# WeebLabs/DSPi

Measured on NVIDIA H100. Metric: audio samples/sec (whole box) at 65536ch x 10-band EQ, 96 kHz; % HBM roofline, higher is better.
Workload: dtype f32

## Files before the change

### dspi_b200/csrc/dspi_common.cuh

```cuda
#pragma once
#ifdef __CUDACC_RTC__
typedef unsigned char uint8_t;
typedef unsigned short uint16_t;
typedef unsigned int uint32_t;
typedef int int32_t;
typedef unsigned long long uint64_t;
typedef long long int64_t;
typedef unsigned long long size_t_rtc;
struct alignas(64) CUtensorMap { unsigned long long opaque[16]; };
#else
#include <cuda.h>
#include <cuda_runtime.h>
#include <stdint.h>
#endif

namespace dspi {

__device__ __forceinline__ uint32_t smem_u32(const void *p)
{
    return static_cast<uint32_t>(__cvta_generic_to_shared(p));
}

__device__ __forceinline__ void mbar_init(uint64_t *bar, uint32_t count)
{
// ... 64 lines not shown
template <int N>
__device__ __forceinline__ void tma_store_wait_read()
{
    asm volatile("cp.async.bulk.wait_group.read %0;" ::"n"(N) : "memory");
}
template <int N>
__device__ __forceinline__ void tma_store_wait_all()
{
    asm volatile("cp.async.bulk.wait_group %0;" ::"n"(N) : "memory");
}

__device__ __forceinline__ void cp_async_4(void *smem_dst, const void *gsrc)
{
    asm volatile("cp.async.ca.shared.global [%0], [%1], 4;" ::"r"(smem_u32(smem_dst)), "l"(gsrc) : "memory");
}
__device__ __forceinline__ void cp_async_commit()
{
    asm volatile("cp.async.commit_group;" ::: "memory");
}
template <int N>
__device__ __forceinline__ void cp_async_wait()
{
    asm volatile("cp.async.wait_group %0;" ::"n"(N) : "memory");
}
__device__ __forceinline__ void cp_async_wait_all()
{
    asm volatile("cp.async.wait_group 0;" ::: "memory");
}
__device__ __forceinline__ void prefetch_tmap(const CUtensorMap *map)
{
    asm volatile("prefetch.tensormap [%0];" ::"l"(reinterpret_cast<uint64_t>(map)) : "memory");
}

}
```

### dspi_b200/csrc/engine.cu

```cuda
#include <cstdarg>
#include <cstdio>
#include <cstdlib>
#include <cstring>
#include <algorithm>
#include <new>
#include <utility>
#include <vector>
#include <sched.h>
#include <unistd.h>
#include <sys/syscall.h>

#include "eq_kernels.cuh"
#include "eq_jit.h"
#include "response.cuh"

namespace {

thread_local char g_err[512] = "";

int fail(int code, const char *fmt, ...)
{
    va_list ap;
    va_start(ap, fmt);
    vsnprintf(g_err, sizeof(g_err), fmt, ap);
// ... 20 lines not shown
        if (cudaGetDriverEntryPoint("cuTensorMapEncodeTiled", &p, cudaEnableDefault, &q) == cudaSuccess && q == cudaDriverEntryPointSuccess)
            fn = reinterpret_cast<EncodeTiledFn>(p);
    }
    return fn;
}

constexpr int kHostBufs = 8;

}

namespace dspi {
char *error_buffer(size_t *cap)
{
    *cap = sizeof(g_err);
    return g_err;
}
}

struct dspi_eq {
    dspi_eq_desc desc;
    int cpl;
    uint32_t rows;
    uint32_t n_groups;
    uint32_t c_pad;
    cudaStream_t stream, s_h2d, s_d2h;
    cudaStream_t s_k[kHostBufs];
    cudaEvent_t ev_begin;
    void *d_aos;
    void *d_coef;
    uint64_t *d_modes;
    uint64_t *d_modes_eff;
    const uint8_t *d_skip;
    uint32_t *d_sched;
    int n_sms;
    size_t aos_elem;
    uint64_t launches;
    void *d_stage[kHostBufs];
    size_t stage_bytes;
    cudaEvent_t ev_in[kHostBufs], ev_done[kHostBufs], ev_out[kHostBufs];
    CUtensorMap tmap;
    void *tm_ptr;
    uint32_t tm_T, tm_ld, tm_rows;
    bool sig_dirty;
    bool sig_stale;
    void *jit;
    char kinfo[320];
    dspi::ResponseBuffers resp;
};

static size_t sched_words(const dspi_eq *e) { return 2 * (size_t)(e->c_pad / 32) + 1; }

extern "C" {

const char *dspi_last_error(void) { return g_err; }

int dspi_device_count(void)
{
    int n = 0;
    if (cudaGetDeviceCount(&n) != cudaSuccess) { cudaGetLastError(); return 0; }
    int ok = 0;
    for (int i = 0; i < n; i++) {
        int major = 0;
        if (cudaDeviceGetAttribute(&major, cudaDevAttrComputeCapabilityMajor, i) == cudaSuccess && major == 9) ok++;
    }
    return ok;
}
// ... 92 lines not shown
    if (!e) return fail(DSPI_ENOMEM, "host allocation failed");
    memset(e, 0, sizeof(*e));
    e->desc = *desc;
    e->sig_dirty = true;
    const bool q28 = desc->arith == DSPI_ARITH_Q28;
    e->cpl = 1;
    if (const char *v = getenv("DSPI_F32_CPL")) e->cpl = atoi(v) == 2 ? 2 : 1;
    if (q28) e->cpl = 1;
    e->rows = 32u * e->cpl;
    e->n_groups = (desc->n_channels + e->rows - 1) / e->rows;
    e->c_pad = e->n_groups * e->rows;
    e->aos_elem = q28 ? sizeof(dspi_biquad_q28) : sizeof(dspi_biquad_f32);

    cudaError_t err;
    const size_t aos_bytes = (size_t)e->c_pad * DSPI_MAX_BANDS * e->aos_elem;
    const size_t coef_bytes = q28 ? (size_t)e->n_groups * DSPI_MAX_BANDS * 20 * 32 * 4 : (size_t)e->c_pad * DSPI_MAX_BANDS * 8 * 4;
    if ((err = cudaStreamCreateWithFlags(&e->stream, cudaStreamNonBlocking)) != cudaSuccess) goto cuda_fail;
    if ((err = cudaStreamCreateWithFlags(&e->s_h2d, cudaStreamNonBlocking)) != cudaSuccess) goto cuda_fail;
    if ((err = cudaStreamCreateWithFlags(&e->s_d2h, cudaStreamNonBlocking)) != cudaSuccess) goto cuda_fail;
    if ((err = cudaEventCreateWithFlags(&e->ev_begin, cudaEventDisableTiming)) != cudaSuccess) goto cuda_fail;
    for (int i = 0; i < kHostBufs; i++) {
        if ((err = cudaStreamCreateWithFlags(&e->s_k[i], cudaStreamNonBlocking)) != cudaSuccess) goto cuda_fail;
        if ((err = cudaEventCreateWithFlags(&e->ev_in[i], cudaEventDisableTiming)) != cudaSuccess) goto cuda_fail;
        if ((err = cudaEventCreateWithFlags(&e->ev_done[i], cudaEventDisableTiming)) != cudaSuccess) goto cuda_fail;
        if ((err = cudaEventCreateWithFlags(&e->ev_out[i], cudaEventDisableTiming)) != cudaSuccess) goto cuda_fail;
    }
    if ((err = cudaMalloc(&e->d_aos, aos_bytes)) != cudaSuccess) goto cuda_fail;
    if ((err = cudaMalloc(&e->d_coef, coef_bytes)) != cudaSuccess) goto cuda_fail;
    if ((err = cudaMemsetAsync(e->d_aos, 0, aos_bytes, e->stream)) != cudaSuccess) goto cuda_fail;
    if ((err = cudaMemsetAsync(e->d_coef, 0, coef_bytes, e->stream)) != cudaSuccess) goto cuda_fail;
    if (!q28) {
        if ((err = cudaMalloc(&e->d_modes, (size_t)e->c_pad * 8)) != cudaSuccess) goto cuda_fail;
        if ((err = cudaMalloc(&e->d_sched, sched_words(e) * 4)) != cudaSuccess) goto cuda_fail;
        if ((err = cudaDeviceGetAttribute(&e->n_sms, cudaDevAttrMultiProcessorCount, desc->device)) != cudaSuccess) goto cuda_fail;
        if ((err = cudaMemsetAsync(e->d_modes, 0, (size_t)e->c_pad * 8, e->stream)) != cudaSuccess) goto cuda_fail;
    }
    if ((err = fill_default_records(e)) != cudaSuccess) goto cuda_fail;
    err = q28 ? dspi::launch_pack_q28((const dspi_biquad_q28 *)e->d_aos, 0, e->c_pad, (int32_t *)e->d_coef, e->stream)
              : dspi::launch_pack_f32((const dspi_biquad_f32 *)e->d_aos, 0, e->c_pad, (float *)e->d_coef, e->d_modes, e->cpl, e->stream);
    if (err != cudaSuccess) goto cuda_fail;
    e->launches++;
    if ((err = cudaStreamSynchronize(e->stream)) != cudaSuccess) goto cuda_fail;
    *out = e;
    return DSPI_OK;

cuda_fail:
    fail(DSPI_ECUDA, "engine setup: %s", cudaGetErrorString(err));
    dspi_eq_destroy(e);
    return err == cudaErrorMemoryAllocation ? DSPI_ENOMEM : DSPI_ECUDA;
}

int dspi_eq_destroy(dspi_eq *e)
{
    if (!e) return DSPI_OK;
    cudaSetDevice(e->desc.device);
    if (e->stream) cudaStreamSynchronize(e->stream);
    if (e->s_h2d) cudaStreamSynchronize(e->s_h2d);
    if (e->s_d2h) cudaStreamSynchronize(e->s_d2h);
    for (int i = 0; i < kHostBufs; i++) {
        if (e->s_k[i]) { cudaStreamSynchronize(e->s_k[i]); cudaStreamDestroy(e->s_k[i]); }
        if (e->d_stage[i]) cudaFree(e->d_stage[i]);
        if (e->ev_in[i]) cudaEventDestroy(e->ev_in[i]);
        if (e->ev_done[i]) cudaEventDestroy(e->ev_done[i]);
        if (e->ev_out[i]) cudaEventDestroy(e->ev_out[i]);
    }
    if (e->d_aos) cudaFree(e->d_aos);
    if (e->d_coef) cudaFree(e->d_coef);
    if (e->d_modes) cudaFree(e->d_modes);
    if (e->d_modes_eff) cudaFree(e->d_modes_eff);
    if (e->d_sched) cudaFree(e->d_sched);
    e->resp.destroy();
    if (e->stream) cudaStreamDestroy(e->stream);
    if (e->s_h2d) cudaStreamDestroy(e->s_h2d);
    if (e->s_d2h) cudaStreamDestroy(e->s_d2h);
    if (e->ev_begin) cudaEventDestroy(e->ev_begin);
    delete e;
    cudaGetLastError();
    return DSPI_OK;
}

static int check_range(dspi_eq *e, uint32_t ch0, uint32_t n, const void *p)
{
    if (!e || !p) return fail(DSPI_EINVAL, "null argument");
    if ((uint64_t)ch0 + n > e->desc.n_channels) return fail(DSPI_ERANGE, "channels [%u, %u) outside engine of %u", ch0, ch0 + n, e->desc.n_channels);
    return DSPI_OK;
}

int dspi_eq_upload_biquads(dspi_eq *e, uint32_t ch0, uint32_t n, const void *biquads)
{
    int rc = check_range(e, ch0, n, biquads);
    if (rc) return rc;
    if (n == 0) return DSPI_OK;
    CU_OK(cudaSetDevice(e->desc.device));
    const size_t row = (size_t)DSPI_MAX_BANDS * e->aos_elem;
    CU_OK(cudaMemcpyAsync((char *)e->d_aos + ch0 * row, biquads, n * row, cudaMemcpyHostToDevice, e->stream));
    if (e->desc.arith == DSPI_ARITH_Q28)
        CU_OK(dspi::launch_pack_q28((const dspi_biquad_q28 *)e->d_aos, ch0, n, (int32_t *)e->d_coef, e->stream));
    else
        CU_OK(dspi::launch_pack_f32((const dspi_biquad_f32 *)e->d_aos, ch0, n, (float *)e->d_coef, e->d_modes, e->cpl, e->stream));
    e->launches++;
    e->sig_dirty = true;
    CU_OK(cudaStreamSynchronize(e->stream));
    return DSPI_OK;
// ... 86 lines not shown
    uint32_t best_n = 0;
    for (uint32_t i = 0; i < cnt;) {
        uint32_t j = i;
        while (j < cnt && sorted[j] == sorted[i]) j++;
        if (j - i > best_n) { best_n = j - i; best = sorted[i]; }
        i = j;
    }
    uint64_t tdf2 = 0;
    for (int b = 0; b < nbt; b++) tdf2 |= (uint64_t)dspi::kModeTdf2 << (4 * b);
    const unsigned pct = (unsigned)(100ull * best_n / cnt);
    if (best == tdf2 && (int)nb == nbt) {
        snprintf(e->kinfo, sizeof(e->kinfo), "aot straight-line biquad (%u%% of sampled channels are all-TDF2); %s", pct, geo);
        return DSPI_OK;
    }
    bool force = false;
    const bool on = dspi::jit::enabled_by_env(&force);
    const char *why = nullptr;
    if (!on) why = "DSPI_JIT=0";
    else if (best == 0) why = "all bands bypassed";
    else if (2 * best_n < cnt) why = "no dominant topology vector";
    else if (!force && C < 1024) why = "engine below 1024 channels (DSPI_JIT=force overrides)";
    if (why) {
        snprintf(e->kinfo, sizeof(e->kinfo), "aot generic column path (%s); %s", why, geo);
        return DSPI_OK;
    }
    char msg[256] = "";
    e->jit = dspi::jit::acquire(best, e->desc.arith == DSPI_ARITH_F32_FUSED, nbt, e->cpl, e->desc.device, msg, sizeof(msg));
    if (e->jit) snprintf(e->kinfo, sizeof(e->kinfo), "jit sig=0x%llx nb=%d (%u%% of sampled channels); %s", (unsigned long long)best, nbt, pct, geo);
    else snprintf(e->kinfo, sizeof(e->kinfo), "aot generic column path (jit unavailable: %.200s); %s", msg, geo);
    return DSPI_OK;
}

static int launch_eq(dspi_eq *e, void *d_samples, uint32_t T, uint32_t ld, uint32_t g0, uint32_t ng, uint32_t n_rows, cudaStream_t stream,
                     uint32_t row_lo = 0)
{
    dspi::EqLaunch a;
    memset(&a, 0, sizeof(a));
    const bool tma_ok = (ld % 4 == 0) && (((uintptr_t)d_samples & 15) == 0);
    if (tma_ok) {
        if (e->tm_ptr != d_samples || e->tm_T != T || e->tm_ld != ld || e->tm_rows != n_rows) {
            int rc = make_tmap(e, d_samples, T, ld, n_rows, &e->tmap);
            if (rc) return rc;
            e->tm_ptr = d_samples; e->tm_T = T; e->tm_ld = ld; e->tm_rows = n_rows;
        }
        a.tmap = e->tmap;
    }
    const bool q28 = e->desc.arith == DSPI_ARITH_Q28;
    a.samples = d_samples;
    a.ld = ld;
    a.coef = q28 ? (void *)((int32_t *)e->d_coef + (size_t)g0 * DSPI_MAX_BANDS * 20 * 32)
                 : (void *)((float *)e->d_coef + (size_t)g0 * DSPI_MAX_BANDS * 8 * 32 * e->cpl);
    const uint64_t *modes = e->d_modes_eff ? e->d_modes_eff : e->d_modes;
    a.modes = modes ? modes + (size_t)g0 * e->rows : nullptr;
    a.n_groups = ng;
    a.sched = e->d_sched + 2 * (((size_t)g0 * e->rows + row_lo) / 32);
    a.n_sms = e->n_sms;
    a.n_rows = n_rows;
    a.row_lo = row_lo;
    a.T = T;
    a.n_bands = e->desc.n_bands;
    a.use_tma = tma_ok ? 1u : 0u;
    if (const char *v = getenv("DSPI_DBG")) a.dbg = (uint32_t)atoi(v);
    cudaError_t err;
    if (e->sig_dirty) {
        int rc = refresh_kernel_choice(e);
        if (rc) return rc;
    }
    if (q28) err = dspi::launch_eq_q28(a, stream);
    else if (e->jit && !(a.dbg & 12u)) {
        char msg[200] = "";
        err = dspi::jit::launch(e->jit, a, stream, msg, sizeof(msg));
        if (err != cudaSuccess) return fail(DSPI_ECUDA, "%s", msg);
    } else err = dspi::launch_eq_f32(a, e->desc.arith == DSPI_ARITH_F32_FUSED, e->cpl, stream);
    if (err != cudaSuccess) return fail(DSPI_ECUDA, "EQ kernel launch: %s", cudaGetErrorString(err));
    e->launches++;
    return DSPI_OK;
}

}

namespace dspi {

static uint32_t range_unit(const dspi_eq *e) { return e->desc.arith == DSPI_ARITH_Q28 ? e->rows : 64u; }

void *eq_aos_mirror(dspi_eq *e) { return e->d_aos; }

static int remask(dspi_eq *e, cudaStream_t s)
{
    if (!e->d_skip) return DSPI_OK;
    if (e->desc.arith == DSPI_ARITH_Q28) {
        CU_OK(launch_skip_q28((int32_t *)e->d_coef, e->d_skip, e->desc.n_channels, s));
        e->launches++;
        return DSPI_OK;
    }
    if (!e->d_modes_eff) {
        CU_OK(cudaMalloc(&e->d_modes_eff, (size_t)e->c_pad * 8));
        CU_OK(cudaMemsetAsync(e->d_modes_eff, 0, (size_t)e->c_pad * 8, s));
    }
    CU_OK(launch_mask_modes(e->d_modes, e->d_skip, e->d_modes_eff, e->desc.n_channels, s));
    e->launches++;
    e->sig_dirty = true;
    return DSPI_OK;
}

int eq_pack_range(dspi_eq *e, uint32_t ch0, uint32_t n, cudaStream_t s, const RoleRange &rr)
{
    if (n == 0) return DSPI_OK;
    CU_OK(cudaSetDevice(e->desc.device));
// ... 144 lines not shown
}

int eq_process_range_on(dspi_eq *e, void *d_rows, uint32_t T, uint32_t ld, uint32_t ch0, uint32_t n, cudaStream_t s)
{
    if (T == 0 || n == 0) return DSPI_OK;
    if (ch0 % 32u) return fail(DSPI_EINVAL, "first channel %u is not a multiple of 32", ch0);
    CU_OK(cudaSetDevice(e->desc.device));
    const uint32_t row_lo = ch0 % e->rows;
    return launch_eq(e, d_rows, T, ld, ch0 / e->rows, (row_lo + n + e->rows - 1) / e->rows, n, s, row_lo);
}

}

extern "C" {

int dspi_eq_kernel_info(dspi_eq *e, char *buf, size_t cap)
{
    if (!e || !buf || cap == 0) return fail(DSPI_EINVAL, "null argument");
    CU_OK(cudaSetDevice(e->desc.device));
    if (e->sig_dirty) {
        int rc = refresh_kernel_choice(e);
        if (rc) return rc;
    }
    snprintf(buf, cap, "%s", e->kinfo);
    return DSPI_OK;
}

int dspi_eq_process_device(dspi_eq *e, void *d_samples, uint32_t T, uint32_t ld)
{
    if (!e || !d_samples) return fail(DSPI_EINVAL, "null argument");
    if (T == 0) return DSPI_OK;
    if (ld < T) return fail(DSPI_EINVAL, "row stride %u < T %u", ld, T);
    CU_OK(cudaSetDevice(e->desc.device));
    return launch_eq(e, d_samples, T, ld, 0, e->n_groups, e->desc.n_channels, e->stream);
}

int dspi_eq_process_device_range(dspi_eq *e, void *d_rows, uint32_t T, uint32_t ld, uint32_t ch0, uint32_t n)
{
    if (!e || !d_rows) return fail(DSPI_EINVAL, "null argument");
    if (T == 0 || n == 0) return DSPI_OK;
    if (ld < T) return fail(DSPI_EINVAL, "row stride %u < T %u", ld, T);
    if ((uint64_t)ch0 + n > e->desc.n_channels) return fail(DSPI_ERANGE, "channels [%u, %u) outside engine of %u", ch0, ch0 + n, e->desc.n_channels);
    if (ch0 % dspi::range_unit(e)) return fail(DSPI_EINVAL, "first channel %u is not a multiple of %u", ch0, dspi::range_unit(e));
    CU_OK(cudaSetDevice(e->desc.device));
    return launch_eq(e, d_rows, T, ld, ch0 / e->rows, (n + e->rows - 1) / e->rows, n, e->stream);
}

}

namespace dspi {
int eq_process_remote_enqueue(dspi_eq *e, void *remote, uint32_t T, uint32_t ch0, uint32_t n_ch)
{
    if (T == 0 || n_ch == 0) return DSPI_OK;
    CU_OK(cudaSetDevice(e->desc.device));
    const uint32_t ld = (T + 3) & ~3u;
    static const size_t chunk_mb_env = [] { const char *v = getenv("DSPI_HOST_CHUNK_MB"); const long n = v ? atol(v) : 0; return (size_t)(n >= 1 && n <= 1024 ? n : 0); }();
    cudaPointerAttributes pa;
    const bool on_device = cudaPointerGetAttributes(&pa, remote) == cudaSuccess && pa.type == cudaMemoryTypeDevice;
    cudaGetLastError();
    const size_t chunk_mb = chunk_mb_env ? chunk_mb_env : (on_device ? 128 : 48);
    uint32_t cc = (uint32_t)((chunk_mb << 20) / ((size_t)ld * 4));
    cc = cc / e->rows * e->rows;
    if (cc < e->rows) cc = e->rows;
    if (cc > e->c_pad) cc = e->c_pad;
    const size_t need = (size_t)cc * ld * 4;
    if (need > e->stage_bytes) {
        CU_OK(cudaStreamSynchronize(e->s_d2h));
// ... 106 lines not shown
```

### dspi_b200/csrc/eq_f32.cu

```cuda
#include "eq_kernels.cuh"
#include "eq_f32_kernel.cuh"

namespace dspi {
namespace {

using namespace core;
using k1::kStageBytes;
using k1::kStages;
using k1::kWarps;

template <typename V, bool FUSED, int NB, bool DYN>
__global__ void __launch_bounds__(kWarps * 32, 1)
eq_f32_kernel(const __grid_constant__ CUtensorMap tmap, float *__restrict__ samples, uint32_t ld, V *__restrict__ coef,
              const uint64_t *__restrict__ modes, uint32_t n_groups, uint32_t n_rows, uint32_t row_lo, uint32_t T, uint32_t nb_active, uint32_t use_tma,
              uint32_t dbg, unsigned long long nz_bits, uint32_t slice_tiles, uint32_t *__restrict__ sched)
{
    k1::eq_f32_body<V, FUSED, NB, DYN, k1::NoSig>(tmap, samples, ld, coef, modes, n_groups, n_rows, row_lo, T, nb_active, use_tma, dbg, nz_bits, slice_tiles, sched);
}

template <typename V, bool FUSED, int NB>
cudaError_t launch_one(const EqLaunch &a, cudaStream_t stream)
{
    constexpr int kTileT = k1::tile_t<V>();
    constexpr size_t smem = (size_t)kWarps * kStages * kStageBytes;
    auto kern = eq_f32_kernel<V, FUSED, NB, false>;
    auto kern_dyn = eq_f32_kernel<V, FUSED, NB, true>;
    static PerDeviceOnce once;
    int dev = 0;
    if (once.needs(&dev)) {
        cudaError_t e = cudaFuncSetAttribute(kern, cudaFuncAttributeMaxDynamicSharedMemorySize, (int)smem);
        if (e == cudaSuccess) e = cudaFuncSetAttribute(kern_dyn, cudaFuncAttributeMaxDynamicSharedMemorySize, (int)smem);
        if (e != cudaSuccess) return e;
        once.mark(dev);
    }
    const uint32_t n_groups = a.n_groups;
    uint32_t grid = (n_groups + kWarps - 1) / kWarps;
    uint32_t slice_tiles = 0;
    uint32_t *sched = nullptr;
    const uint32_t ntiles = (a.T + kTileT - 1) / kTileT;
    if (a.sched && a.use_tma && a.T >= 1024 && (a.dbg & 8u)) {
        slice_tiles = 512 / kTileT;
        sched = a.sched;
        if (grid > (uint32_t)a.n_sms) grid = a.n_sms;
        else if (grid < (uint32_t)a.n_sms && (uint32_t)a.n_sms * kWarps <= n_groups * ((ntiles + slice_tiles - 1) / slice_tiles)) grid = a.n_sms;
        cudaError_t e = cudaMemsetAsync(sched, 0, (size_t)(1 + n_groups) * sizeof(uint32_t), stream);
        if (e != cudaSuccess) return e;
    }
    if (sched)
        kern_dyn<<<grid, kWarps * 32, smem, stream>>>(a.tmap, (float *)a.samples, a.ld, (V *)a.coef, a.modes, n_groups, a.n_rows, a.row_lo, a.T, a.n_bands, a.use_tma,
                                                      a.dbg, 0x8000000080000000ull, slice_tiles, sched);
    else
        kern<<<grid, kWarps * 32, smem, stream>>>(a.tmap, (float *)a.samples, a.ld, (V *)a.coef, a.modes, n_groups, a.n_rows, a.row_lo, a.T, a.n_bands, a.use_tma,
                                                  a.dbg, 0x8000000080000000ull, 0u, nullptr);
    return cudaGetLastError();
}

template <typename V, bool FUSED>
cudaError_t launch_nb(const EqLaunch &a, cudaStream_t stream)
{
    if (a.n_bands <= 10) return launch_one<V, FUSED, 10>(a, stream);
    return launch_one<V, FUSED, 12>(a, stream);
}

}

cudaError_t launch_eq_f32(const EqLaunch &a, bool fused, int cpl, cudaStream_t stream)
{
    if (cpl == 2) return fused ? launch_nb<P2, true>(a, stream) : launch_nb<P2, false>(a, stream);
    return fused ? launch_nb<float, true>(a, stream) : launch_nb<float, false>(a, stream);
}

__global__ void pack_f32_kernel(const dspi_biquad_f32 *__restrict__ aos, uint32_t ch0, uint32_t n, float *__restrict__ coef,
                                uint64_t *__restrict__ modes, int cpl, RoleRange rr)
{
    const uint32_t i = blockIdx.x * blockDim.x + threadIdx.x;
    if (i >= n || (rr.reject && rr.reject[i])) return;
    const uint32_t ch = ch0 + blockIdx.y * rr.stride + (rr.inst ? rr.inst[i] : i);
    const uint32_t rows = 32 * cpl;
    const uint32_t g = ch / rows, r = ch % rows, lane = r & 31, h = r >> 5;
    uint64_t mw = 0;
    for (int b = 0; b < kMaxBands; b++) {
        const dspi_biquad_f32 &q = aos[(size_t)ch * kMaxBands + b];
        float v[8];
        uint32_t mode;
        if (q.bypass) mode = kModeBypass;
        else if (!q.use_svf) mode = kModeTdf2;
// ... 60 lines not shown
```

### dspi_b200/csrc/eq_f32_jit_entry.cuh

```cuda
#include "eq_f32_kernel.cuh"

#ifndef DSPI_JIT_NB
#define DSPI_JIT_NB 10
#endif
#if DSPI_JIT_CPL == 2
typedef dspi::core::P2 JitV;
#else
typedef float JitV;
#endif

extern "C" __global__ void __launch_bounds__(dspi::k1::kWarps * 32, 1)
eq_f32_jit(const __grid_constant__ CUtensorMap tmap, float *__restrict__ samples, uint32_t ld, JitV *__restrict__ coef,
           const uint64_t *__restrict__ modes, uint32_t n_groups, uint32_t n_rows, uint32_t row_lo, uint32_t T, uint32_t nb_active, uint32_t use_tma, uint32_t dbg,
           unsigned long long nz_bits, uint32_t slice_tiles, uint32_t *__restrict__ sched)
{
    dspi::k1::eq_f32_body<JitV, (DSPI_JIT_FUSED) != 0, DSPI_JIT_NB, false, dspi::k1::SigWord<(DSPI_JIT_SIG)>>(
        tmap, samples, ld, coef, modes, n_groups, n_rows, row_lo, T, nb_active, use_tma, dbg, nz_bits, slice_tiles, sched);
}
```

### dspi_b200/csrc/eq_f32_kernel.cuh

```cuda
#pragma once
#include "eq_core.cuh"

namespace dspi {
namespace k1 {

using namespace core;

constexpr int kStages = 3;
constexpr int kWarps = 8;
constexpr uint32_t kStageBytes = 8192;
template <typename V> __host__ __device__ constexpr int tile_t() { return 64 / Lanes<V>::CPL; }
template <typename V> __host__ __device__ constexpr int sub_t() { return tile_t<V>() / 4; }

__device__ __forceinline__ uint32_t chunk_off(int r, int k, uint32_t half_bytes)
{
    return (uint32_t)(k >> 3) * half_bytes + r * 128 + ((((k & 7) ^ (r & 7))) << 4);
}

struct NoSig { static constexpr bool enabled = false; static constexpr unsigned long long word = 0; };
template <unsigned long long W> struct SigWord { static constexpr bool enabled = true; static constexpr unsigned long long word = W; };

template <typename V, bool FUSED, int NB, bool DYN, typename SIG>
__device__ __forceinline__ void eq_f32_body(const CUtensorMap &tmap, float *__restrict__ samples, uint32_t ld, V *__restrict__ coef,
              const uint64_t *__restrict__ modes, uint32_t n_groups, uint32_t n_rows, uint32_t row_lo, uint32_t T, uint32_t nb_active, uint32_t use_tma, uint32_t dbg, unsigned long long nz_bits, uint32_t slice_tiles, uint32_t *__restrict__ sched)
{
    constexpr int CPL = Lanes<V>::CPL;
    constexpr int kRows = 32 * CPL;
    constexpr int kTileT = tile_t<V>();
    constexpr int kSub = sub_t<V>();
    constexpr int kHalves = kTileT / 32;
    constexpr uint32_t kHalfBytes = kRows * 128;
    static_assert(kRows * kTileT * 4 == (int)kStageBytes, "every geometry fills the same 8 KB stage");

    extern __shared__ __align__(1024) uint8_t smem_raw[];
    __shared__ uint64_t bars[kWarps][kStages];

    const int warp = threadIdx.x >> 5, lane = threadIdx.x & 31;

    uint8_t *my_smem = smem_raw + (size_t)warp * kStages * kStageBytes;
    uint64_t *full = bars[warp];
    if (lane == 0) {
        if (use_tma) prefetch_tmap(&tmap);
        for (int s = 0; s < kStages; s++) mbar_init(&full[s], 1);
        fence_mbar_init();
    }
    __syncwarp();

    const V nz = v_bits<V>(nz_bits);
    const uint32_t ntiles = (T + kTileT - 1) / kTileT;
    const bool mem_on = !(dbg & 2u);

    const uint32_t n_slices = DYN ? (ntiles + slice_tiles - 1) / slice_tiles : 1;
    const uint32_t n_items = DYN ? n_groups * n_slices : 0;
    uint32_t tcount = 0;
    for (;;) {
        uint32_t g, tile_begin, tile_end, slice = 0;
        if constexpr (DYN) {
            uint32_t item = 0;
            if (lane == 0) item = atomicAdd(&sched[0], 1u);
            item = __shfl_sync(0xffffffffu, item, 0);
            if (item >= n_items) break;
            slice = item / n_groups;
            g = item - slice * n_groups;
            tile_begin = slice * slice_tiles;
            tile_end = min(ntiles, tile_begin + slice_tiles);
            if (slice > 0) {
                if (lane == 0) {
                    const volatile uint32_t *flag = sched + 1 + g;
                    while (*flag < slice) __nanosleep(100);
                    __threadfence();
// ... 135 lines not shown
                        tma_store_wait_read<1>();
                        issue_load(nxt, tcount + kStages - 1);
                    }
                }
            } else {
                __syncwarp();
                for (int r = 0; r < kRows; r++) {
                    const uint32_t ch = c0 + r;
                    for (int h = 0; h < kHalves; h++) {
                        const uint32_t t = tile * kTileT + h * 32 + lane;
                        const float v = *reinterpret_cast<const float *>(buf + chunk_off(r, h * 8 + (lane >> 2), kHalfBytes) + ((lane & 3) << 2));
                        if (t < T && ch < n_rows) samples[(size_t)ch * ld + t] = v;
                    }
                }
                __syncwarp();
            }
        }


        if (!tma) tcount = tcount0;
        int h_lo = 0, h_hi = 0;
#pragma unroll
        for (int h = 0; h < CPL; h++) {
            if (c0 + 32 * h + lane < 0) h_lo = h + 1;
            if ((uint32_t)(c0 + 32 * h + lane) < n_rows) h_hi = h + 1;
        }
        bank.store(my_coef, h_lo, h_hi, DYN);
        if constexpr (!DYN) break;
        __threadfence();
        __syncwarp();
        if (lane == 0) atomicExch(&sched[1 + g], slice + 1);
    }
    if (use_tma && lane == 0) tma_store_wait_all<0>();
}


}
}
```

### dspi_b200/csrc/eq_jit.cu

```cuda
#include "eq_kernels.cuh"
#include "eq_f32_kernel.cuh"
#include "eq_jit.h"

#include <dlfcn.h>
#include <mutex>
#include <stdio.h>
#include <string.h>
#include <string>
#include <vector>

#include "jit_headers.inc"

namespace dspi {
namespace jit {
namespace {

typedef struct _nvrtcProgram *nvrtcProgram;
struct Nvrtc {
    void *so = nullptr;
    int (*CreateProgram)(nvrtcProgram *, const char *, const char *, int, const char *const *, const char *const *) = nullptr;
    int (*CompileProgram)(nvrtcProgram, int, const char *const *) = nullptr;
    int (*DestroyProgram)(nvrtcProgram *) = nullptr;
    int (*GetCUBINSize)(nvrtcProgram, size_t *) = nullptr;
    int (*GetCUBIN)(nvrtcProgram, char *) = nullptr;
    int (*GetProgramLogSize)(nvrtcProgram, size_t *) = nullptr;
    int (*GetProgramLog)(nvrtcProgram, char *) = nullptr;
    const char *(*GetErrorString)(int) = nullptr;
    bool ok = false;
};

Nvrtc &nvrtc()
{
    static Nvrtc n;
    static bool tried = false;
    if (tried) return n;
    tried = true;
    const char *names[] = { "libnvrtc.so.12", "libnvrtc.so", "/usr/local/cuda/lib64/libnvrtc.so.12", "/usr/local/cuda/lib64/libnvrtc.so" };
    for (const char *nm : names) {
        n.so = dlopen(nm, RTLD_NOW | RTLD_LOCAL);
        if (n.so) break;
    }
    if (!n.so) return n;
#define SYM(f) *(void **)(&n.f) = dlsym(n.so, "nvrtc" #f)
    SYM(CreateProgram); SYM(CompileProgram); SYM(DestroyProgram); SYM(GetCUBINSize); SYM(GetCUBIN);
    SYM(GetProgramLogSize); SYM(GetProgramLog); SYM(GetErrorString);
#undef SYM
    n.ok = n.CreateProgram && n.CompileProgram && n.DestroyProgram && n.GetCUBINSize && n.GetCUBIN && n.GetProgramLogSize && n.GetProgramLog;
    return n;
}

struct Driver {
    decltype(&cuLibraryLoadData) LibraryLoadData = nullptr;
    decltype(&cuLibraryGetKernel) LibraryGetKernel = nullptr;
    decltype(&cuKernelSetAttribute) KernelSetAttribute = nullptr;
    decltype(&cuLaunchKernel) LaunchKernel = nullptr;
    decltype(&cuGetErrorString) GetErrorString = nullptr;
    bool ok = false;
};

Driver &driver()
{
    static Driver d;
    static bool tried = false;
    if (tried) return d;
    tried = true;
    auto get = [](const char *name) -> void * {
        void *p = nullptr;
        cudaDriverEntryPointQueryResult q;
        if (cudaGetDriverEntryPoint(name, &p, cudaEnableDefault, &q) != cudaSuccess || q != cudaDriverEntryPointSuccess) { cudaGetLastError(); return nullptr; }
        return p;
    };
    d.LibraryLoadData = (decltype(d.LibraryLoadData))get("cuLibraryLoadData");
    d.LibraryGetKernel = (decltype(d.LibraryGetKernel))get("cuLibraryGetKernel");
    d.KernelSetAttribute = (decltype(d.KernelSetAttribute))get("cuKernelSetAttribute");
    d.LaunchKernel = (decltype(d.LaunchKernel))get("cuLaunchKernel");
    d.GetErrorString = (decltype(d.GetErrorString))get("cuGetErrorString");
    d.ok = d.LibraryLoadData && d.LibraryGetKernel && d.KernelSetAttribute && d.LaunchKernel;
    return d;
}

std::string cu_err(CUresult r)
{
    const char *s = nullptr;
    if (driver().GetErrorString) driver().GetErrorString(r, &s);
    char b[96];
    snprintf(b, sizeof(b), "%s (%d)", s ? s : "CUDA driver error", (int)r);
    return b;
}

struct Entry {
    uint64_t sig;
    bool fused;
    int nb;
    int cpl;
    CUlibrary lib;
    CUkernel kern;
    uint64_t smem_set;
    std::string fail;
};

std::mutex g_mu;
std::vector<Entry *> g_cache;

constexpr int kWarps = k1::kWarps;
constexpr size_t kSmem = (size_t)kWarps * k1::kStages * k1::kStageBytes;

Entry *compile(uint64_t sig, bool fused, int nb, int cpl)
{
    Entry *en = new Entry{ sig, fused, nb, cpl, nullptr, nullptr, 0, "" };
    Nvrtc &n = nvrtc();
    Driver &d = driver();
    if (!n.ok) { en->fail = "libnvrtc not available"; return en; }
    if (!d.ok) { en->fail = "driver lacks cuLibraryLoadData/cuLibraryGetKernel"; return en; }
    nvrtcProgram prog = nullptr;
    int rc = n.CreateProgram(&prog, "#include \"eq_f32_jit_entry.cuh\"\n", "dspi_eq_jit.cu", kJitHeaderCount, kJitHeaderSrc, kJitHeaderNames);
    if (rc != 0) { en->fail = "nvrtcCreateProgram failed"; return en; }
    char dsig[64], dfused[32], dnb[32], dcpl[32];
    snprintf(dsig, sizeof(dsig), "-DDSPI_JIT_SIG=0x%llxull", (unsigned long long)sig);
    snprintf(dfused, sizeof(dfused), "-DDSPI_JIT_FUSED=%d", fused ? 1 : 0);
    snprintf(dnb, sizeof(dnb), "-DDSPI_JIT_NB=%d", nb);
    snprintf(dcpl, sizeof(dcpl), "-DDSPI_JIT_CPL=%d", cpl);
    const char *opts[] = { "--gpu-architecture=sm_90a", "-std=c++17", "-ftz=true", "-prec-div=true", "-prec-sqrt=true", "-fmad=false",
                           "-lineinfo", dsig, dfused, dnb, dcpl };
    rc = n.CompileProgram(prog, (int)(sizeof(opts) / sizeof(opts[0])), opts);
    if (rc != 0) {
        size_t ls = 0;
        n.GetProgramLogSize(prog, &ls);
        std::string log(ls ? ls : 1, '\0');
        if (ls) n.GetProgramLog(prog, &log[0]);
        if (log.size() > 400) log.resize(400);
        en->fail = std::string("nvrtcCompileProgram: ") + (n.GetErrorString ? n.GetErrorString(rc) : "error") + ": " + log;
        n.DestroyProgram(&prog);
        return en;
    }
    size_t sz = 0;
    std::vector<char> cubin;
    if (n.GetCUBINSize(prog, &sz) != 0 || sz == 0) { en->fail = "nvrtcGetCUBINSize failed"; n.DestroyProgram(&prog); return en; }
    cubin.resize(sz);
    if (n.GetCUBIN(prog, cubin.data()) != 0) { en->fail = "nvrtcGetCUBIN failed"; n.DestroyProgram(&prog); return en; }
    n.DestroyProgram(&prog);
    CUresult r = d.LibraryLoadData(&en->lib, cubin.data(), nullptr, nullptr, 0, nullptr, nullptr, 0);
    if (r != CUDA_SUCCESS) { en->fail = "cuLibraryLoadData: " + cu_err(r); return en; }
    r = d.LibraryGetKernel(&en->kern, en->lib, "eq_f32_jit");
    if (r != CUDA_SUCCESS) { en->fail = "cuLibraryGetKernel: " + cu_err(r); en->kern = nullptr; return en; }
    return en;
}
// ... 17 lines not shown
    for (Entry *e : g_cache)
        if (e->sig == sig && e->fused == fused && e->nb == nb && e->cpl == cpl) { en = e; break; }
    if (!en) {
        en = compile(sig, fused, nb, cpl);
        g_cache.push_back(en);
    }
    if (!en->fail.empty()) {
        if (msg && cap) snprintf(msg, cap, "%s", en->fail.c_str());
        return nullptr;
    }
    if (device >= 0 && device < 64 && !((en->smem_set >> device) & 1)) {
        CUdevice dev = device;
        CUresult r = driver().KernelSetAttribute(CU_FUNC_ATTRIBUTE_MAX_DYNAMIC_SHARED_SIZE_BYTES, (int)kSmem, en->kern, dev);
        if (r != CUDA_SUCCESS) {
            if (msg && cap) snprintf(msg, cap, "cuKernelSetAttribute: %s", cu_err(r).c_str());
            return nullptr;
        }
        en->smem_set |= 1ull << device;
    }
    return en;
}

cudaError_t launch(void *handle, const EqLaunch &a, cudaStream_t stream, char *msg, size_t cap)
{
    Entry *en = (Entry *)handle;
    CUtensorMap tmap = a.tmap;
    float *samples = (float *)a.samples;
    uint32_t ld = a.ld;
    void *coef = a.coef;
    const uint64_t *modes = a.modes;
    uint32_t n_groups = a.n_groups, n_rows = a.n_rows, row_lo = a.row_lo, T = a.T, nb_active = a.n_bands, use_tma = a.use_tma, dbg = a.dbg, slice_tiles = 0;
    unsigned long long nz = 0x8000000080000000ull;
    uint32_t *sched = nullptr;
    void *args[] = { &tmap, &samples, &ld, &coef, &modes, &n_groups, &n_rows, &row_lo, &T, &nb_active, &use_tma, &dbg, &nz, &slice_tiles, &sched };
    const uint32_t grid = (n_groups + kWarps - 1) / kWarps;
    CUresult r = driver().LaunchKernel((CUfunction)en->kern, grid, 1, 1, kWarps * 32, 1, 1, (unsigned)kSmem, (CUstream)stream, args, nullptr);
    if (r != CUDA_SUCCESS) {
        if (msg && cap) snprintf(msg, cap, "cuLaunchKernel(eq_f32_jit): %s", cu_err(r).c_str());
        return cudaErrorLaunchFailure;
    }
    return cudaSuccess;
}

}
}
```

### dspi_b200/csrc/eq_kernels.cuh

```cuda
#pragma once
#include <utility>
#include <vector>

#include "eq_modes.cuh"
#include "dspi_b200.h"

namespace dspi {

static_assert(kMaxBands == DSPI_MAX_BANDS, "band stride");

struct EqLaunch {
    CUtensorMap tmap;
    void *samples;
    uint32_t ld;
    void *coef;
    const uint64_t *modes;
    uint32_t n_groups;
    uint32_t n_rows;
    uint32_t row_lo;
    uint32_t T;
    uint32_t n_bands;
    uint32_t use_tma;
    uint32_t dbg;
    uint32_t *sched;
    int n_sms;
};

struct PerDeviceOnce {
    unsigned long long done = 0;
    bool needs(int *device_out)
    {
        int dev = 0;
        cudaGetDevice(&dev);
        *device_out = dev;
        return dev < 0 || dev >= 64 || !((done >> dev) & 1ull);
    }
    void mark(int dev) { if (dev >= 0 && dev < 64) done |= 1ull << dev; }
};

char *error_buffer(size_t *cap);

struct RoleRange {
    uint32_t roles = 1, stride = 0;
    const int32_t *reject = nullptr;
    const float *fs = nullptr;
    const uint32_t *inst = nullptr;
    const uint16_t *band_mask = nullptr;
};

cudaError_t launch_eq_f32(const EqLaunch &a, bool fused, int cpl, cudaStream_t stream);
cudaError_t launch_pack_f32(const dspi_biquad_f32 *aos, uint32_t ch0, uint32_t n, float *coef, uint64_t *modes, int cpl, cudaStream_t stream,
                            const RoleRange &rr = RoleRange());
cudaError_t launch_unpack_f32(dspi_biquad_f32 *aos, uint32_t ch0, uint32_t n, const float *coef, int cpl, cudaStream_t stream,
                              const RoleRange &rr = RoleRange());

cudaError_t launch_eq_q28(const EqLaunch &a, cudaStream_t stream);
cudaError_t launch_pack_q28(const dspi_biquad_q28 *aos, uint32_t ch0, uint32_t n, int32_t *coef, cudaStream_t stream, const RoleRange &rr = RoleRange());
cudaError_t launch_unpack_q28(dspi_biquad_q28 *aos, uint32_t ch0, uint32_t n, const int32_t *coef, cudaStream_t stream,
// ... 32 lines not shown
```

### dspi_b200/csrc/eq_modes.cuh

```cuda
#pragma once
#include "dspi_common.cuh"

namespace dspi {

constexpr int kMaxBands = 12;

enum : uint32_t {
    kModeBypass = 0,
    kModeTdf2   = 1,
    kModeSvfLP  = 2,
    kModeSvfHP  = 3,
    kModeSvfPK  = 4,
    kModeSvfSH  = 5
};

}
```

Before: 335.6 billion.

## Chain consecutive EQ launches with PDL and per-group release flags

Launches the non-dynamic f32 EQ kernel with programmatic stream serialization so that the next launch can start while the previous one is still draining. Each warp group waits on a per-group sequence flag published with release semantics by the previous launch, falling back to griddepcontrol.wait once the whole previous grid has finished. This targets the launch gap and tail between back-to-back full-channel process calls. In exchange it adds spin-waiting with nanosleep, extra fences, and more complex cross-launch ordering that must stay correct.

```diff
diff --git a/dspi_b200/csrc/dspi_common.cuh b/dspi_b200/csrc/dspi_common.cuh
--- a/dspi_b200/csrc/dspi_common.cuh
+++ b/dspi_b200/csrc/dspi_common.cuh
@@ -120,4 +120,33 @@
     asm volatile("prefetch.tensormap [%0];" ::"l"(reinterpret_cast<uint64_t>(map)) : "memory");
 }
 
+__device__ __forceinline__ void griddep_launch_dependents()
+{
+    asm volatile("griddepcontrol.launch_dependents;" ::: "memory");
 }
+__device__ __forceinline__ void griddep_wait()
+{
+    asm volatile("griddepcontrol.wait;" ::: "memory");
+}
+
+__device__ __forceinline__ void fence_proxy_async_global()
+{
+    asm volatile("fence.proxy.async.global;" ::: "memory");
+}
+
+__device__ __forceinline__ uint32_t ld_acquire_gpu(const uint32_t *p)
+{
+    uint32_t v;
+    asm volatile("ld.acquire.gpu.global.u32 %0, [%1];" : "=r"(v) : "l"(p) : "memory");
+    return v;
+}
+__device__ __forceinline__ void st_release_gpu(uint32_t *p, uint32_t v)
+{
+    asm volatile("st.release.gpu.global.u32 [%0], %1;" ::"l"(p), "r"(v) : "memory");
+}
+__device__ __forceinline__ void red_add_release_gpu(uint32_t *p, uint32_t v)
+{
+    asm volatile("red.release.gpu.global.add.u32 [%0], %1;" ::"l"(p), "r"(v) : "memory");
+}
+
+}
diff --git a/dspi_b200/csrc/engine.cu b/dspi_b200/csrc/engine.cu
--- a/dspi_b200/csrc/engine.cu
+++ b/dspi_b200/csrc/engine.cu
@@ -76,6 +76,8 @@
     uint64_t *d_modes_eff;
     const uint8_t *d_skip;
     uint32_t *d_sched;
+    uint32_t *d_chain;
+    uint32_t chain_seq, chain_prev, chain_done;
     int n_sms;
     size_t aos_elem;
     uint64_t launches;
@@ -234,6 +236,9 @@
     if (!q28) {
         if ((err = cudaMalloc(&e->d_modes, (size_t)e->c_pad * 8)) != cudaSuccess) goto cuda_fail;
         if ((err = cudaMalloc(&e->d_sched, sched_words(e) * 4)) != cudaSuccess) goto cuda_fail;
+        if ((err = cudaMalloc(&e->d_chain, (1 + (size_t)e->n_groups) * 4)) != cudaSuccess) goto cuda_fail;
+        if ((err = cudaMemsetAsync(e->d_chain, 0, (1 + (size_t)e->n_groups) * 4, e->stream)) != cudaSuccess) goto cuda_fail;
+        e->chain_seq = 1;
         if ((err = cudaDeviceGetAttribute(&e->n_sms, cudaDevAttrMultiProcessorCount, desc->device)) != cudaSuccess) goto cuda_fail;
         if ((err = cudaMemsetAsync(e->d_modes, 0, (size_t)e->c_pad * 8, e->stream)) != cudaSuccess) goto cuda_fail;
     }
@@ -271,6 +276,7 @@
     if (e->d_modes) cudaFree(e->d_modes);
     if (e->d_modes_eff) cudaFree(e->d_modes_eff);
     if (e->d_sched) cudaFree(e->d_sched);
+    if (e->d_chain) cudaFree(e->d_chain);
     e->resp.destroy();
     if (e->stream) cudaStreamDestroy(e->stream);
     if (e->s_h2d) cudaStreamDestroy(e->s_h2d);
@@ -423,7 +429,7 @@
 }
 
 static int launch_eq(dspi_eq *e, void *d_samples, uint32_t T, uint32_t ld, uint32_t g0, uint32_t ng, uint32_t n_rows, cudaStream_t stream,
-                     uint32_t row_lo = 0)
+                     uint32_t row_lo = 0, bool chain = false)
 {
     dspi::EqLaunch a;
     memset(&a, 0, sizeof(a));
@@ -452,6 +458,8 @@
     a.n_bands = e->desc.n_bands;
     a.use_tma = tma_ok ? 1u : 0u;
     if (const char *v = getenv("DSPI_DBG")) a.dbg = (uint32_t)atoi(v);
+    chain = chain && !q28 && tma_ok && !(a.dbg & 24u);
+    if (chain) a.chain = dspi::K1Chain{ e->d_chain, e->chain_seq, e->chain_prev, e->chain_done };
     cudaError_t err;
     if (e->sig_dirty) {
         int rc = refresh_kernel_choice(e);
@@ -465,6 +473,11 @@
     } else err = dspi::launch_eq_f32(a, e->desc.arith == DSPI_ARITH_F32_FUSED, e->cpl, stream);
     if (err != cudaSuccess) return fail(DSPI_ECUDA, "EQ kernel launch: %s", cudaGetErrorString(err));
     e->launches++;
+    if (chain) {
+        e->chain_prev = e->chain_seq;
+        e->chain_done += ng;
+        if (++e->chain_seq == 0) e->chain_seq = 1;
+    } else e->chain_prev = 0;
     return DSPI_OK;
 }
 
@@ -675,7 +688,7 @@
     if (T == 0) return DSPI_OK;
     if (ld < T) return fail(DSPI_EINVAL, "row stride %u < T %u", ld, T);
     CU_OK(cudaSetDevice(e->desc.device));
-    return launch_eq(e, d_samples, T, ld, 0, e->n_groups, e->desc.n_channels, e->stream);
+    return launch_eq(e, d_samples, T, ld, 0, e->n_groups, e->desc.n_channels, e->stream, 0, true);
 }
 
 int dspi_eq_process_device_range(dspi_eq *e, void *d_rows, uint32_t T, uint32_t ld, uint32_t ch0, uint32_t n)
diff --git a/dspi_b200/csrc/eq_f32.cu b/dspi_b200/csrc/eq_f32.cu
--- a/dspi_b200/csrc/eq_f32.cu
+++ b/dspi_b200/csrc/eq_f32.cu
@@ -13,9 +13,10 @@
 __global__ void __launch_bounds__(kWarps * 32, 1)
 eq_f32_kernel(const __grid_constant__ CUtensorMap tmap, float *__restrict__ samples, uint32_t ld, V *__restrict__ coef,
               const uint64_t *__restrict__ modes, uint32_t n_groups, uint32_t n_rows, uint32_t row_lo, uint32_t T, uint32_t nb_active, uint32_t use_tma,
-              uint32_t dbg, unsigned long long nz_bits, uint32_t slice_tiles, uint32_t *__restrict__ sched)
+              uint32_t dbg, unsigned long long nz_bits, uint32_t slice_tiles, uint32_t *__restrict__ sched, const K1Chain chain)
 {
-    k1::eq_f32_body<V, FUSED, NB, DYN, k1::NoSig>(tmap, samples, ld, coef, modes, n_groups, n_rows, row_lo, T, nb_active, use_tma, dbg, nz_bits, slice_tiles, sched);
+    k1::eq_f32_body<V, FUSED, NB, DYN, k1::NoSig>(tmap, samples, ld, coef, modes, n_groups, n_rows, row_lo, T, nb_active, use_tma, dbg, nz_bits, slice_tiles, sched,
+                                                  chain);
 }
 
 template <typename V, bool FUSED, int NB>
@@ -48,10 +49,21 @@
     }
     if (sched)
         kern_dyn<<<grid, kWarps * 32, smem, stream>>>(a.tmap, (float *)a.samples, a.ld, (V *)a.coef, a.modes, n_groups, a.n_rows, a.row_lo, a.T, a.n_bands, a.use_tma,
-                                                      a.dbg, 0x8000000080000000ull, slice_tiles, sched);
-    else
-        kern<<<grid, kWarps * 32, smem, stream>>>(a.tmap, (float *)a.samples, a.ld, (V *)a.coef, a.modes, n_groups, a.n_rows, a.row_lo, a.T, a.n_bands, a.use_tma,
-                                                  a.dbg, 0x8000000080000000ull, 0u, nullptr);
+                                                      a.dbg, 0x8000000080000000ull, slice_tiles, sched, K1Chain{});
+    else {
+        cudaLaunchAttribute attr;
+        attr.id = cudaLaunchAttributeProgrammaticStreamSerialization;
+        attr.val.programmaticStreamSerializationAllowed = 1;
+        cudaLaunchConfig_t cfg = {};
+        cfg.gridDim = dim3(grid);
+        cfg.blockDim = dim3(kWarps * 32);
+        cfg.dynamicSmemBytes = smem;
+        cfg.stream = stream;
+        cfg.attrs = &attr;
+        cfg.numAttrs = a.chain.seq ? 1 : 0;
+        return cudaLaunchKernelEx(&cfg, kern, a.tmap, (float *)a.samples, a.ld, (V *)a.coef, a.modes, n_groups, a.n_rows, a.row_lo, a.T, a.n_bands, a.use_tma,
+                                  a.dbg, 0x8000000080000000ull, 0u, (uint32_t *)nullptr, a.chain);
+    }
     return cudaGetLastError();
 }
 
diff --git a/dspi_b200/csrc/eq_f32_jit_entry.cuh b/dspi_b200/csrc/eq_f32_jit_entry.cuh
--- a/dspi_b200/csrc/eq_f32_jit_entry.cuh
+++ b/dspi_b200/csrc/eq_f32_jit_entry.cuh
@@ -12,8 +12,8 @@
 extern "C" __global__ void __launch_bounds__(dspi::k1::kWarps * 32, 1)
 eq_f32_jit(const __grid_constant__ CUtensorMap tmap, float *__restrict__ samples, uint32_t ld, JitV *__restrict__ coef,
            const uint64_t *__restrict__ modes, uint32_t n_groups, uint32_t n_rows, uint32_t row_lo, uint32_t T, uint32_t nb_active, uint32_t use_tma, uint32_t dbg,
-           unsigned long long nz_bits, uint32_t slice_tiles, uint32_t *__restrict__ sched)
+           unsigned long long nz_bits, uint32_t slice_tiles, uint32_t *__restrict__ sched, const dspi::K1Chain chain)
 {
     dspi::k1::eq_f32_body<JitV, (DSPI_JIT_FUSED) != 0, DSPI_JIT_NB, false, dspi::k1::SigWord<(DSPI_JIT_SIG)>>(
-        tmap, samples, ld, coef, modes, n_groups, n_rows, row_lo, T, nb_active, use_tma, dbg, nz_bits, slice_tiles, sched);
+        tmap, samples, ld, coef, modes, n_groups, n_rows, row_lo, T, nb_active, use_tma, dbg, nz_bits, slice_tiles, sched, chain);
 }
diff --git a/dspi_b200/csrc/eq_f32_kernel.cuh b/dspi_b200/csrc/eq_f32_kernel.cuh
--- a/dspi_b200/csrc/eq_f32_kernel.cuh
+++ b/dspi_b200/csrc/eq_f32_kernel.cuh
@@ -20,10 +20,33 @@
 struct NoSig { static constexpr bool enabled = false; static constexpr unsigned long long word = 0; };
 template <unsigned long long W> struct SigWord { static constexpr bool enabled = true; static constexpr unsigned long long word = W; };
 
+__device__ __forceinline__ void chain_wait(const K1Chain &ch, uint32_t g)
+{
+    if (ch.prev_seq != 0 && (int32_t)(ld_acquire_gpu(ch.words) - ch.prev_done) < 0) {
+        while ((int32_t)(ld_acquire_gpu(ch.words + 1 + g) - ch.prev_seq) < 0) __nanosleep(256);
+        fence_proxy_async_global();
+    } else {
+        griddep_wait();
+    }
+}
+
+__device__ __forceinline__ void chain_publish(const K1Chain &ch, uint32_t g, int lane)
+{
+    __threadfence();
+    __syncwarp();
+    if (lane == 0) {
+        fence_proxy_async_global();
+        st_release_gpu(ch.words + 1 + g, ch.seq);
+        red_add_release_gpu(ch.words, 1u);
+    }
+}
+
 template <typename V, bool FUSED, int NB, bool DYN, typename SIG>
 __device__ __forceinline__ void eq_f32_body(const CUtensorMap &tmap, float *__restrict__ samples, uint32_t ld, V *__restrict__ coef,
-              const uint64_t *__restrict__ modes, uint32_t n_groups, uint32_t n_rows, uint32_t row_lo, uint32_t T, uint32_t nb_active, uint32_t use_tma, uint32_t dbg, unsigned long long nz_bits, uint32_t slice_tiles, uint32_t *__restrict__ sched)
-{
+              const uint64_t *__restrict__ modes, uint32_t n_groups, uint32_t n_rows, uint32_t row_lo, uint32_t T, uint32_t nb_active, uint32_t use_tma, uint32_t dbg, unsigned long long nz_bits, uint32_t slice_tiles, uint32_t *__restrict__ sched,
+              const K1Chain &chain)
+{
+    if (chain.seq) griddep_launch_dependents();
     constexpr int CPL = Lanes<V>::CPL;
     constexpr int kRows = 32 * CPL;
     constexpr int kTileT = tile_t<V>();
@@ -36,6 +59,7 @@
     __shared__ uint64_t bars[kWarps][kStages];
 
     const int warp = threadIdx.x >> 5, lane = threadIdx.x & 31;
+    if (!DYN && chain.seq && lane == 0 && blockIdx.x * kWarps + warp < n_groups) chain_wait(chain, blockIdx.x * kWarps + warp);
 
     uint8_t *my_smem = smem_raw + (size_t)warp * kStages * kStageBytes;
     uint64_t *full = bars[warp];
@@ -237,8 +261,9 @@
         if (lane == 0) atomicExch(&sched[1 + g], slice + 1);
     }
     if (use_tma && lane == 0) tma_store_wait_all<0>();
-}
-
-
-}
-}
+    if (!DYN && chain.seq && blockIdx.x * kWarps + warp < n_groups) chain_publish(chain, blockIdx.x * kWarps + warp, lane);
+}
+
+
+}
+}
diff --git a/dspi_b200/csrc/eq_jit.cu b/dspi_b200/csrc/eq_jit.cu
--- a/dspi_b200/csrc/eq_jit.cu
+++ b/dspi_b200/csrc/eq_jit.cu
@@ -53,7 +53,7 @@
     decltype(&cuLibraryLoadData) LibraryLoadData = nullptr;
     decltype(&cuLibraryGetKernel) LibraryGetKernel = nullptr;
     decltype(&cuKernelSetAttribute) KernelSetAttribute = nullptr;
-    decltype(&cuLaunchKernel) LaunchKernel = nullptr;
+    decltype(&cuLaunchKernelEx) LaunchKernelEx = nullptr;
     decltype(&cuGetErrorString) GetErrorString = nullptr;
     bool ok = false;
 };
@@ -73,9 +73,9 @@
     d.LibraryLoadData = (decltype(d.LibraryLoadData))get("cuLibraryLoadData");
     d.LibraryGetKernel = (decltype(d.LibraryGetKernel))get("cuLibraryGetKernel");
     d.KernelSetAttribute = (decltype(d.KernelSetAttribute))get("cuKernelSetAttribute");
-    d.LaunchKernel = (decltype(d.LaunchKernel))get("cuLaunchKernel");
+    d.LaunchKernelEx = (decltype(d.LaunchKernelEx))get("cuLaunchKernelEx");
     d.GetErrorString = (decltype(d.GetErrorString))get("cuGetErrorString");
-    d.ok = d.LibraryLoadData && d.LibraryGetKernel && d.KernelSetAttribute && d.LaunchKernel;
+    d.ok = d.LibraryLoadData && d.LibraryGetKernel && d.KernelSetAttribute && d.LaunchKernelEx;
     return d;
 }
 
@@ -111,7 +111,7 @@
     Nvrtc &n = nvrtc();
     Driver &d = driver();
     if (!n.ok) { en->fail = "libnvrtc not available"; return en; }
-    if (!d.ok) { en->fail = "driver lacks cuLibraryLoadData/cuLibraryGetKernel"; return en; }
+    if (!d.ok) { en->fail = "driver lacks cuLibraryLoadData/cuLibraryGetKernel/cuLaunchKernelEx"; return en; }
     nvrtcProgram prog = nullptr;
     int rc = n.CreateProgram(&prog, "#include \"eq_f32_jit_entry.cuh\"\n", "dspi_eq_jit.cu", kJitHeaderCount, kJitHeaderSrc, kJitHeaderNames);
     if (rc != 0) { en->fail = "nvrtcCreateProgram failed"; return en; }
@@ -195,11 +195,23 @@
     uint32_t n_groups = a.n_groups, n_rows = a.n_rows, row_lo = a.row_lo, T = a.T, nb_active = a.n_bands, use_tma = a.use_tma, dbg = a.dbg, slice_tiles = 0;
     unsigned long long nz = 0x8000000080000000ull;
     uint32_t *sched = nullptr;
-    void *args[] = { &tmap, &samples, &ld, &coef, &modes, &n_groups, &n_rows, &row_lo, &T, &nb_active, &use_tma, &dbg, &nz, &slice_tiles, &sched };
-    const uint32_t grid = (n_groups + kWarps - 1) / kWarps;
-    CUresult r = driver().LaunchKernel((CUfunction)en->kern, grid, 1, 1, kWarps * 32, 1, 1, (unsigned)kSmem, (CUstream)stream, args, nullptr);
+    K1Chain chain = a.chain;
+    void *args[] = { &tmap, &samples, &ld, &coef, &modes, &n_groups, &n_rows, &row_lo, &T, &nb_active, &use_tma, &dbg, &nz, &slice_tiles, &sched, &chain };
+    CUlaunchAttribute attr;
+    attr.id = CU_LAUNCH_ATTRIBUTE_PROGRAMMATIC_STREAM_SERIALIZATION;
+    attr.value.programmaticStreamSerializationAllowed = 1;
+    CUlaunchConfig cfg = {};
+    cfg.gridDimX = (n_groups + kWarps - 1) / kWarps;
+    cfg.gridDimY = cfg.gridDimZ = 1;
+    cfg.blockDimX = kWarps * 32;
+    cfg.blockDimY = cfg.blockDimZ = 1;
+    cfg.sharedMemBytes = (unsigned)kSmem;
+    cfg.hStream = (CUstream)stream;
+    cfg.attrs = &attr;
+    cfg.numAttrs = chain.seq ? 1 : 0;
+    CUresult r = driver().LaunchKernelEx(&cfg, (CUfunction)en->kern, args, nullptr);
     if (r != CUDA_SUCCESS) {
-        if (msg && cap) snprintf(msg, cap, "cuLaunchKernel(eq_f32_jit): %s", cu_err(r).c_str());
+        if (msg && cap) snprintf(msg, cap, "cuLaunchKernelEx(eq_f32_jit): %s", cu_err(r).c_str());
         return cudaErrorLaunchFailure;
     }
     return cudaSuccess;
diff --git a/dspi_b200/csrc/eq_kernels.cuh b/dspi_b200/csrc/eq_kernels.cuh
--- a/dspi_b200/csrc/eq_kernels.cuh
+++ b/dspi_b200/csrc/eq_kernels.cuh
@@ -24,6 +24,7 @@
     uint32_t dbg;
     uint32_t *sched;
     int n_sms;
+    K1Chain chain;
 };
 
 struct PerDeviceOnce {
diff --git a/dspi_b200/csrc/eq_modes.cuh b/dspi_b200/csrc/eq_modes.cuh
--- a/dspi_b200/csrc/eq_modes.cuh
+++ b/dspi_b200/csrc/eq_modes.cuh
@@ -14,4 +14,11 @@
     kModeSvfSH  = 5
 };
 
+struct K1Chain {
+    uint32_t *words;
+    uint32_t seq;
+    uint32_t prev_seq;
+    uint32_t prev_done;
+};
+
 }
```

Measured after the change: 344.5 billion, median of 6. 2.7% higher.
